# donydchen/matchnerf

Hardware: AMD Instinct MI355X
Metric: rendered rays/sec (3-view, 64 samples/ray) (higher is better)
Workload: dtype f32; 1 GPU

## Files before the change

### include/mnerf.h

```cpp
#ifndef MNERF_H_
#define MNERF_H_

#include <stdint.h>

#ifdef __cplusplus
extern "C" {
#endif

#define MNERF_ABI_VERSION 12
#define MNERF_MAX_VIEWS 16
#define MNERF_FEAT_CH 128
#define MNERF_COND_STRIDE_MAX 96
#define MNERF_COND_STRIDE_MAX_F32 64

enum {
  MNERF_OK = 0,
  MNERF_E_NULL = -1,
  MNERF_E_RANGE = -2,
  MNERF_E_UNSUPPORTED = -3,
  MNERF_E_ALIGN = -4
};

typedef struct mnerf_view {
  float extr[12];
// ... 167 lines not shown
int mnerf_window_attention_backward(const float* q, const float* k, const float* v, const float* out, const float* g_out,
                                    float* g_q, float* g_k, float* g_v, int32_t batch, int32_t h, int32_t w,
                                    int32_t num_splits, int32_t shifted, void* workspace, size_t workspace_bytes,
                                    void* stream);
int mnerf_window_attention_presplit_stats(const float* q, const float* k, const float* v, float* out, float* row_stats,
                                          int32_t batch, int32_t h, int32_t w, int32_t num_splits, int32_t shifted,
                                          void* workspace, size_t workspace_bytes, void* stream);
int mnerf_window_attention_backward_stats(const float* q, const float* k, const float* v, const float* out, const float* g_out,
                                          const float* row_stats, float* g_q, float* g_k, float* g_v, int32_t batch, int32_t h,
                                          int32_t w, int32_t num_splits, int32_t shifted, void* workspace,
                                          size_t workspace_bytes, void* stream);

int mnerf_instance_norm(const float* x, const float* residual, float* out, int64_t planes, int64_t plane_size,
                        float eps, int32_t relu_inner, int32_t relu_outer, float* out_absmax, void* stream);

int mnerf_instance_norm_backward(const float* x, const float* dy, float* dx, int64_t planes, int64_t plane_size, float eps,
                                 int32_t relu, void* stream);

int mnerf_upsample_bilinear2x(const float* in, const float* add, float* out, int64_t planes, int32_t h, int32_t w, void* stream);
int mnerf_upsample_bilinear2x_backward(const float* dout, float* din, int64_t planes, int32_t h, int32_t w, void* stream);

#define MNERF_ABSMAX_SLOTS 64
#define MNERF_ABSMAX_STRIDE 32
#define MNERF_ABSMAX_FLOATS (MNERF_ABSMAX_SLOTS * MNERF_ABSMAX_STRIDE)
typedef struct mnerf_conv {
  const float* wstream;
  int64_t wstream_floats;
  const float* bias;
  int32_t c_in, c_out, ksize, stride;
  int32_t ew;
  float leaky_slope;
} mnerf_conv;
int64_t mnerf_conv_wstream_floats(int32_t c_in, int32_t c_out, int32_t ksize);
#define MNERF_CONV_OUT_NCHW 0
#define MNERF_CONV_OUT_CHANNEL_LAST 1
#define MNERF_CONV_OUT_PAIR_MAJOR 2
int mnerf_conv2d(const mnerf_conv* cv, const float* in, int32_t in_channels_last, int32_t upsample2x,
                 const float* in_absmax, const float* add_bilinear2x, const float* add_channel_last, float* out,
                 int32_t out_layout, float* out_absmax, int32_t n_img, int32_t h_in, int32_t w_in, void* stream);
int64_t mnerf_conv_stem_wstream_floats(void);
int mnerf_conv_stem(const float* wstream, int32_t ew, const float* in, const float* in_absmax, float* out,
                    int32_t n_img, int32_t h_in, int32_t w_in, void* stream);
int mnerf_absmax(const float* x, int64_t n, float* out, void* stream);

int mnerf_conv2d_backward_data(const float* dy, const float* w_tap_major, float* dx, int32_t n_img, int32_t c_in, int32_t c_out,
                               int32_t h_in, int32_t w_in, int32_t ksize, int32_t stride, void* stream);
size_t mnerf_conv2d_backward_weight_workspace_bytes(int32_t n_img, int32_t c_in, int32_t c_out, int32_t h_in, int32_t w_in,
                                                    int32_t ksize, int32_t stride);
int mnerf_conv2d_backward_weight(const float* x, const float* dy, float* dw, void* workspace, size_t workspace_bytes, int32_t n_img,
                                 int32_t c_in, int32_t c_out, int32_t h_in, int32_t w_in, int32_t ksize, int32_t stride, void* stream);
int mnerf_conv2d_backward_weight_f16x3(const float* x, const float* dy, const float* x_absmax, const float* dy_absmax, float* dw,
                                       void* workspace, size_t workspace_bytes, int32_t n_img, int32_t c_in, int32_t c_out, int32_t h_in,
                                       int32_t w_in, int32_t ksize, int32_t stride, void* stream);
int mnerf_conv2d_forward_f32(const float* x, const float* w_tap_major, const float* bias, float* y, int32_t n_img, int32_t c_in,
                             int32_t c_out, int32_t h_in, int32_t w_in, int32_t ksize, int32_t stride, void* stream);
size_t mnerf_conv_stem_backward_weight_workspace_bytes(int32_t n_img, int32_t h_in, int32_t w_in);
int mnerf_conv_stem_backward_weight(const float* x, const float* dy, float* dw, void* workspace, size_t workspace_bytes, int32_t n_img,
// ... 89 lines not shown
```

### matchnerf_amd/csrc/conv.hip

```cpp
#include "split_f16.hpp"

#define CONV_NW 4
#define CONV_BUF_BYTES 36864u

#ifdef CONV_TIMELINE
#define CONV_TL_POINTS 6
#define CONV_TL_ITERS 64
#define CONV_TL_STAMP(k)                                                                                       \
  do {                                                                                                         \
    __builtin_amdgcn_sched_barrier(0);                                                                         \
    if (tl_out && iter < CONV_TL_ITERS) tl_out[iter * CONV_TL_POINTS + (k)] = __builtin_amdgcn_s_memtime();    \
    __builtin_amdgcn_sched_barrier(0);                                                                         \
  } while (0)
#else
#define CONV_TL_STAMP(k) do {} while (0)
#endif
struct ConvParams {
  unsigned long long* tl;
  const float* in;
  const float* wstream;
  const float* bias;
  float* out;
  const float* in_absmax;
  float* out_absmax;
// ... 320 lines not shown
  p.out_layout = out_layout;
  p.add_cl = add_channel_last;
  MNERF_REQUIRE(out_layout == MNERF_CONV_OUT_NCHW || mnerf_aligned16(out), MNERF_E_ALIGN,
                "%s: a channel-last output must be 16-byte aligned", who);
  MNERF_REQUIRE(out_layout != MNERF_CONV_OUT_PAIR_MAJOR || n_img % 2 == 0, MNERF_E_RANGE,
                "%s: pair-major output needs an even number of images, got %d", who, n_img);
  MNERF_REQUIRE(!add_channel_last || (out_layout != MNERF_CONV_OUT_NCHW && mnerf_aligned16(add_channel_last)), MNERF_E_RANGE,
                "%s: add_channel_last needs a channel-last output layout and a 16-byte aligned tile", who);
  const long long n_pix = (long long)n_img * p.h_out * p.w_out;
  const int tpw = (n_pix + 255) / 256 >= 256 ? 2 : 1;
  const long long per_wg = 32 * tpw * CONV_NW;
  const dim3 grid((unsigned)((n_pix + per_wg - 1) / per_wg));
  const size_t lds = 2 * CONV_BUF_BYTES;
  hipStream_t st = (hipStream_t)stream;
  const bool cl = in_channels_last != 0;
  MNERF_REQUIRE(!cl || nmb == 4, MNERF_E_UNSUPPORTED, "%s: channel-last input is built for c_out = 128 only", who);
#define CONV_CASE(NMB, TPW, CLV)                                                                                      \
  if (nmb == NMB && tpw == TPW && cl == CLV) {                                                                        \
    static std::atomic<unsigned long long> attr{0};                                                                   \
    if (mnerf_once_per_device(attr))                                                                                  \
      (void)hipFuncSetAttribute((const void*)conv_kernel<NMB, TPW, CLV>, hipFuncAttributeMaxDynamicSharedMemorySize,   \
                                (int)lds);                                                                            \
    hipLaunchKernelGGL((conv_kernel<NMB, TPW, CLV>), grid, dim3(CONV_NW * 64), lds, st, p);                           \
  }
  CONV_CASE(2, 2, false) CONV_CASE(2, 1, false) CONV_CASE(3, 2, false) CONV_CASE(3, 1, false)
  CONV_CASE(4, 2, false) CONV_CASE(4, 1, false) CONV_CASE(4, 2, true) CONV_CASE(4, 1, true)
#undef CONV_CASE
  return mnerf_check_launch(who);
}

#define STEM_STEPS 10
#define STEM_K 147
#define STEM_W_BYTES (STEM_STEPS * 2 * H16_UNIT_BYTES)

struct StemParams {
  const float* in;
  const float* wstream;
  float* out;
  const float* in_absmax;
  int n_img, h_in, w_in, h_out, w_out, ew;
};

__global__ __launch_bounds__(CONV_NW * 64, 2) void conv_stem_kernel(StemParams P) {
  extern __shared__ __attribute__((aligned(16))) float stem_smem[];
  const unsigned buf0 = (unsigned)(size_t)(__attribute__((address_space(3))) float*)stem_smem;
  int* tab_off = reinterpret_cast<int*>(stem_smem) + STEM_W_BYTES / 4;
  int* tab_dy = tab_off + 16 * STEM_STEPS;
  int* tab_dx = tab_dy + 16 * STEM_STEPS;
  const int tid = threadIdx.x, lane = tid & 63;
  const int wave = __builtin_amdgcn_readfirstlane(tid >> 6);
  const int n = lane & 31, hl = lane >> 5;
  {
    const float* src = P.wstream + lane * 4;
    glds_segment(src, buf0, STEM_W_BYTES / 1024, wave, CONV_NW);
  }
  const int hw_in = P.h_in * P.w_in;
  for (int k = tid; k < 16 * STEM_STEPS; k += CONV_NW * 64) {
    const int tap = k / 3, c = k - 3 * tap, dy = tap / 7 - 3, dx = tap % 7 - 3;
    const bool real = k < STEM_K;
    tab_off[k] = real ? c * hw_in + dy * P.w_in + dx : 0;
    tab_dy[k] = real ? dy : 100;
    tab_dx[k] = real ? dx : 100;
  }
  const int hw_out = P.h_out * P.w_out;
  const long long n_pix = (long long)P.n_img * hw_out;
  constexpr int TPW = 2;
  int cy[TPW], cx[TPW];
  long long ibase[TPW], obase[TPW];
  bool live[TPW];
#pragma unroll
  for (int t = 0; t < TPW; ++t) {
    const long long p = ((long long)blockIdx.x * CONV_NW + wave) * (32 * TPW) + t * 32 + n;
    live[t] = p < n_pix;
    const long long pc = live[t] ? p : n_pix - 1;
    const int img = (int)(pc / hw_out), rem = (int)(pc - (long long)img * hw_out);
    const int oy = rem / P.w_out, ox = rem - oy * P.w_out;
    cy[t] = 2 * oy;
    cx[t] = 2 * ox;
    ibase[t] = (long long)img * 3 * hw_in + (long long)cy[t] * P.w_in + cx[t];
    obase[t] = (long long)img * 64 * hw_out + rem;
  }
  const int eg = gain_exp(mnerf_absmax_read(P.in_absmax));
  const float mult = pow2i(eg);
  f32x16 acc[TPW][2];
#pragma unroll
  for (int t = 0; t < TPW; ++t) acc[t][0] = acc[t][1] = (f32x16)(0.0f);
  segment_wait();
  __syncthreads();

// ... 40 lines not shown
#pragma unroll
    for (int m = 0; m < 2; ++m) {
      const f16x8 ah = __builtin_bit_cast(f16x8, a[m * 128]), al = __builtin_bit_cast(f16x8, a[m * 128 + 64]);
#pragma unroll
      for (int t = 0; t < TPW; ++t) acc[t][m] = mfma16h(ah, b[t].lo, acc[t][m]);
#pragma unroll
      for (int t = 0; t < TPW; ++t) acc[t][m] = mfma16h(al, b[t].hi, acc[t][m]);
#pragma unroll
      for (int t = 0; t < TPW; ++t) acc[t][m] = mfma16h(ah, b[t].hi, acc[t][m]);
    }
  }
  const float cm = pow2i(-(P.ew + eg));
#pragma unroll
  for (int t = 0; t < TPW; ++t) {
    if (!live[t]) continue;
#pragma unroll
    for (int m = 0; m < 2; ++m)
#pragma unroll
      for (int r = 0; r < 16; ++r)
        P.out[obase[t] + (long long)(32 * m + 8 * (r >> 2) + 4 * hl + (r & 3)) * hw_out] = acc[t][m][r] * cm;
  }
}

extern "C" int64_t mnerf_conv_stem_wstream_floats(void) { return STEM_W_BYTES / 4; }

extern "C" int mnerf_conv_stem(const float* wstream, int32_t ew, const float* in, const float* in_absmax, float* out,
                               int32_t n_img, int32_t h_in, int32_t w_in, void* stream) {
  const char* who = "mnerf_conv_stem";
  MNERF_REQUIRE(n_img >= 0 && h_in >= 1 && w_in >= 1, MNERF_E_RANGE, "%s: n_img=%d h_in=%d w_in=%d", who, n_img, h_in, w_in);
  MNERF_REQUIRE((long long)3 * h_in * w_in <= 0x7fffffffLL, MNERF_E_RANGE, "%s: image too large", who);
  if (n_img == 0) return MNERF_OK;
  MNERF_REQUIRE(wstream && in && in_absmax && out, MNERF_E_NULL, "%s: NULL buffer", who);
  MNERF_REQUIRE(mnerf_aligned16(wstream), MNERF_E_ALIGN, "%s: wstream must be 16-byte aligned", who);
  StemParams p;
  p.in = in;
  p.wstream = wstream;
  p.out = out;
  p.in_absmax = in_absmax;
  p.n_img = n_img;
  p.h_in = h_in;
  p.w_in = w_in;
  p.h_out = (h_in + 6 - 7) / 2 + 1;
  p.w_out = (w_in + 6 - 7) / 2 + 1;
  p.ew = ew;
  const long long n_pix = (long long)n_img * p.h_out * p.w_out;
  const size_t lds = STEM_W_BYTES + 3 * 16 * STEM_STEPS * sizeof(int);
  static std::atomic<unsigned long long> attr{0};
  if (mnerf_once_per_device(attr))
    (void)hipFuncSetAttribute((const void*)conv_stem_kernel, hipFuncAttributeMaxDynamicSharedMemorySize, (int)lds);
  hipLaunchKernelGGL(conv_stem_kernel, dim3((unsigned)((n_pix + 255) / 256)), dim3(CONV_NW * 64), lds, (hipStream_t)stream, p);
  return mnerf_check_launch(who);
}
```

### matchnerf_amd/csrc/instance_norm.hip

```cpp
#include "common.hpp"

template <int THREADS>
__device__ __forceinline__ float in_block_sum(float v, float* red) {
#pragma unroll
  for (int off = 32; off > 0; off >>= 1) v += __shfl_xor(v, off, 64);
  const int wave = threadIdx.x >> 6;
  __syncthreads();
  if ((threadIdx.x & 63) == 0) red[wave] = v;
  __syncthreads();
  float t = 0.0f;
#pragma unroll
  for (int i = 0; i < THREADS / 64; ++i) t += red[i];
  return t;
}

__device__ __forceinline__ float in_finish(float x, float mean, float rstd, float res, bool has_res, int relu_inner,
                                           int relu_outer) {
  float v = (x - mean) * rstd;
  if (relu_inner) v = fmaxf(v, 0.0f);
  if (has_res) v += res;
  if (relu_outer) v = fmaxf(v, 0.0f);
  return v;
}

// ... 106 lines not shown
  const bool vec = (n & 3) == 0 && mnerf_aligned16(x) && mnerf_aligned16(out) && (!residual || mnerf_aligned16(residual));
  const dim3 grid((unsigned)planes);
#define IN_LAUNCH(T, V)                                                                                              \
  hipLaunchKernelGGL((instance_norm_cached_kernel<T, V>), grid, dim3(T), 0, st, x, residual, out, n, eps, relu_inner, \
                     relu_outer, out_absmax)
  if (vec && n <= 256 * 8 * 4) IN_LAUNCH(256, 8);
  else if (vec && n <= 256 * 20 * 4) IN_LAUNCH(256, 20);
  else if (vec && n <= 512 * 40 * 4) IN_LAUNCH(512, 40);
  else
    hipLaunchKernelGGL(instance_norm_stream_kernel, grid, dim3(256), 0, st, x, residual, out, n, eps, relu_inner, relu_outer,
                       out_absmax);
#undef IN_LAUNCH
  return mnerf_check_launch("mnerf_instance_norm");
}

__global__ __launch_bounds__(512) void instance_norm_backward_kernel(const float* __restrict__ x, const float* __restrict__ dy, float* __restrict__ dx,
                                                                     int plane_size, float eps, int relu) {
  __shared__ float red[8];
  const size_t base = (size_t)blockIdx.x * plane_size;
  const float* xs = x + base;
  const float* gs = dy + base;
  const float inv_n = 1.0f / (float)plane_size;
  float s = 0.0f;
  for (int j = threadIdx.x; j < plane_size; j += 512) s += xs[j];
  const float mean = in_block_sum<512>(s, red) * inv_n;
  float q = 0.0f;
  for (int j = threadIdx.x; j < plane_size; j += 512) {
    const float a = xs[j] - mean;
    q += a * a;
  }
// ... 178 lines not shown
```

### matchnerf_amd/gmflow.py

```python
import math
import os

import torch
import torch.nn as nn
import torch.nn.functional as F

from . import hip
from .autograd import window_attention
from .camera import pair_list


def _fused_norm(x):
    return x.is_cuda and not torch.is_grad_enabled()


def _train_hip(x):
    import os
    return (x.is_cuda and x.dtype == torch.float32 and torch.is_grad_enabled()
            and os.environ.get("MNERF_TRAIN_CNN", "hip") != "torch")


def _train_packs(owner, convs, device):
    import os
    if os.environ.get("MNERF_TRAIN_CNN", "hip") == "f32":
# ... 58 lines not shown
    return hip.conv2d(x, ws, bias, conv.in_channels, conv.out_channels, conv.kernel_size[0], conv.stride[0], ew, in_absmax, **kw)


class ResidualBlock(nn.Module):

    def __init__(self, in_planes, planes, stride=1):
        super().__init__()
        self.conv1 = nn.Conv2d(in_planes, planes, 3, stride=stride, padding=1, bias=False)
        self.conv2 = nn.Conv2d(planes, planes, 3, padding=1, bias=False)
        self.stride = stride
        if stride != 1 or in_planes != planes:
            self.downsample = nn.Sequential(nn.Conv2d(in_planes, planes, 1, stride=stride))
        else:
            self.downsample = None

    def forward_fused(self, x, x_absmax, scal):
        y = _hip_conv(self.conv1, x, x_absmax)
        hip.instance_norm(y, relu_inner=True, out=y, out_absmax=scal[0])
        y = _hip_conv(self.conv2, y, scal[0])
        if self.downsample is not None:
            x = _hip_conv(self.downsample[0], x, x_absmax)
            hip.instance_norm(x, out=x)
        hip.instance_norm(y, residual=x, relu_inner=True, relu_outer=True, out=y, out_absmax=scal[1])
        return y, scal[1]

    def forward(self, x):
        if _train_hip(x):
            from . import autograd as AG
            y = AG.instance_norm(AG.conv2d(self.conv1, x), relu=True)
            y = AG.instance_norm(AG.conv2d(self.conv2, y), relu=True)
            if self.downsample is not None:
                x = AG.instance_norm(AG.conv2d(self.downsample[0], x))
            return F.relu(x + y)
        y = F.relu(F.instance_norm(self.conv1(x)))
        y = F.relu(F.instance_norm(self.conv2(y)))
        if self.downsample is not None:
            x = F.instance_norm(self.downsample(x))
        return F.relu(x + y)


class CNNEncoder(nn.Module):

    def __init__(self, output_dim=128):
        super().__init__()
        self.conv1 = nn.Conv2d(3, 64, 7, stride=2, padding=3, bias=False)
        self.layer1 = nn.Sequential(ResidualBlock(64, 64, 1), ResidualBlock(64, 64, 1))
        self.layer2 = nn.Sequential(ResidualBlock(64, 96, 2), ResidualBlock(96, 96, 1))
        self.layer3 = nn.Sequential(ResidualBlock(96, 128, 2), ResidualBlock(128, 128, 1))
        self.conv2 = nn.Conv2d(128, output_dim, 1)
        for m in self.modules():
            if isinstance(m, nn.Conv2d):
                nn.init.kaiming_normal_(m.weight, mode="fan_out", nonlinearity="relu")

    def forward(self, x, tokens_plus=None):
        if _fused_norm(x):
            scal = hip.absmax_regions(14, x.device)
            x = x.contiguous()
            hip.absmax(x, scal[13])
            key = (int(self.conv1.weight._version), int(self.conv1.weight.data_ptr()), str(x.device))
            if getattr(self, "_stem_pack", None) is None or self._stem_pack[0] != key:
                ws, ew = pack_conv_stem(self.conv1.weight)
                self._stem_pack = (key, torch.from_numpy(ws).to(x.device), ew)
            x = hip.conv_stem(x, self._stem_pack[1], self._stem_pack[2], scal[13])
            hip.instance_norm(x, relu_inner=True, out=x, out_absmax=scal[0])
            amax, k = scal[0], 1
            for layer in (self.layer1, self.layer2, self.layer3):
                for blk in layer:
                    x, amax = blk.forward_fused(x, amax, scal[k:k + 2])
                    k += 2
            if tokens_plus is not None:
                return _hip_conv(self.conv2, x, amax, out_layout=hip.CONV_OUT_CHANNEL_LAST, add_channel_last=tokens_plus)
            return _hip_conv(self.conv2, x, amax)
        if _train_hip(x):
            from . import autograd as AG
            convs = [m for m in self.modules() if isinstance(m, nn.Conv2d)]
            _train_packs(self, convs, x.device)
            x = AG.instance_norm(AG.conv2d(self.conv1, x), relu=True)
            x = AG.conv2d(self.conv2, self.layer3(self.layer2(self.layer1(x))))
            _drop_train_packs(convs)
        else:
            x = F.relu(F.instance_norm(self.conv1(x)))
            x = self.conv2(self.layer3(self.layer2(self.layer1(x))))
        return x if tokens_plus is None else x.permute(0, 2, 3, 1) + tokens_plus.reshape(x.shape[2], x.shape[3], -1)


EB_SEG_FLOATS = 32 * 256
EB_CHUNK = 128
# ... 251 lines not shown
            else:
                right = F.interpolate(right, scale_factor=2, mode="bilinear", align_corners=False) + conv(self.conv_l2rs[i + 1], left)
        if _train_hip(x):
            _drop_train_packs(list(self.conv_ls) + list(self.conv_l2rs))
        return right


_SINE_CACHE = {}
_PAIR_INDEX_CACHE = {}


def _pair_index_tensors(v, device):
    key = (int(v), str(device))
    if key not in _PAIR_INDEX_CACHE:
        pairs = pair_list(v)
        _PAIR_INDEX_CACHE[key] = (torch.tensor([a for a, _ in pairs], device=device),
                                  torch.tensor([bb for _, bb in pairs], device=device))
    return _PAIR_INDEX_CACHE[key]


def sine_position_tokens(h, w, channels, device):
    key = (h, w, channels, str(device))
    if key not in _SINE_CACHE:
        npf = channels // 2
        y = (torch.arange(1, h + 1, dtype=torch.float32) / (h + 1e-6) * (2 * math.pi))[:, None].expand(h, w)
        x = (torch.arange(1, w + 1, dtype=torch.float32) / (w + 1e-6) * (2 * math.pi))[None, :].expand(h, w)
        i = torch.arange(npf, dtype=torch.float32)
        dim_t = 10000.0 ** (2 * torch.div(i, 2, rounding_mode="trunc") / npf)

        def emb(t):
            a = t[..., None] / dim_t
            return torch.stack([a[..., 0::2].sin(), a[..., 1::2].cos()], -1).flatten(-2)
# ... 56 lines not shown
        pe = sine_position_tokens(h // splits, w // splits, ch, x.device).repeat(splits, splits, 1).reshape(h * w, ch).contiguous()
        tok = self.backbone((x - self._mean) / self._std, tokens_plus=pe)
        if tuple(tok.shape[1:]) != (h, w, ch):
            raise ValueError(f"backbone output {tuple(tok.shape[1:])} != expected {(h, w, ch)} for a {hh}x{ww} input")
        return tok.reshape(b, n_v, h, w, ch)

    def pair_maps(self, tokens, pairs=None, attn_splits_list=None, wo_self_attn=False):
        b, v, h, w, ch = tokens.shape
        splits = self._splits(attn_splits_list)
        pairs_all = pair_list(v)
        p0, p_n = self._contiguous_range(pairs, len(pairs_all), "pair_maps pairs")
        if p_n == 0:
            up = 2 ** self.featup_net.n_blocks
            return [tokens.new_empty(b, 0, 2, h, w, ch), tokens.new_empty(b, 0, 2, up * h, up * w, ch)]
        tok = tokens.reshape(b, v, h * w, ch)
        ia, ib = _pair_index_tensors(v, tok.device)
        if p_n != len(pairs_all):
            ia, ib = ia[p0:p0 + p_n], ib[p0:p0 + p_n]
        outs0, outs1 = [], []
        for bi in range(b):
            src = torch.cat([tok[bi, ia], tok[bi, ib]], 0).contiguous()
            src = self.transformer(src, p_n, h, w, splits, wo_self_attn)
            outs0.append(torch.stack([src[:p_n], src[p_n:]], 1).reshape(p_n, 2, h, w, ch))
            if _fused_norm(src) and self.featup_net.n_blocks >= 1:
                outs1.append(self.featup_net.forward_tokens(src.reshape(2 * p_n, h, w, ch), pair_major=True))
            else:
                up = self.featup_net(src.reshape(2 * p_n, h, w, ch).permute(0, 3, 1, 2))
                up = up.permute(0, 2, 3, 1)
                outs1.append(torch.stack([up[:p_n], up[p_n:]], 1).contiguous())
        if b == 1:
            return [outs0[0].unsqueeze(0).contiguous(), outs1[0].unsqueeze(0).contiguous()]
        return [torch.stack(outs0, 0).contiguous(), torch.stack(outs1, 0).contiguous()]


def pair_major_to_view_chunks(feat_pm):
    b, p_n = feat_pm.shape[:2]
# ... 7 lines not shown
```

### matchnerf_amd/hip.py

```python
import contextlib
import ctypes as C
import os

import numpy as np

MNERF_ABI_VERSION = 12
MNERF_POSE_FLOATS = 24
MNERF_OK, MNERF_E_NULL, MNERF_E_RANGE, MNERF_E_UNSUPPORTED, MNERF_E_ALIGN = 0, -1, -2, -3, -4
MNERF_MAX_VIEWS = 16
MNERF_COND_STRIDE_MAX, MNERF_COND_STRIDE_MAX_F32 = 96, 64
SMALL_FIXED = 32

_LIB = None
_LIB_PATH = os.environ.get("MNERF_LIB") or os.path.join(os.path.dirname(os.path.abspath(__file__)), "libmnerf_hip.so")

EXPORTS = ("mnerf_abi_version", "mnerf_last_error", "mnerf_struct_size", "mnerf_ray_samples", "mnerf_composite", "mnerf_cost_volume",
           "mnerf_cost_volume_operand_bytes", "mnerf_cost_volume_operands",
           "mnerf_composite_backward", "mnerf_cost_volume_backward", "mnerf_decoder_backward", "mnerf_decoder_backward_workspace_bytes", "mnerf_debug_set_knob",
           "mnerf_decoder_wstream_floats", "mnerf_decoder_chunk", "mnerf_decoder_samples", "mnerf_render_workspace_bytes",
           "mnerf_render_chunk", "mnerf_render_chunk_fused", "mnerf_render_chunk_is_fused", "mnerf_render_takes_pose_table", "mnerf_window_attention",
           "mnerf_window_attention_presplit", "mnerf_window_attention_workspace_bytes", "mnerf_window_attention_backward", "mnerf_window_attention_backward_workspace_bytes", "mnerf_qkv_projection", "mnerf_qkv_wstream_floats", "mnerf_qkv_window_images", "mnerf_window_attention_images", "mnerf_instance_norm", "mnerf_instance_norm_backward", "mnerf_upsample_bilinear2x", "mnerf_upsample_bilinear2x_backward", "mnerf_conv2d", "mnerf_conv_wstream_floats", "mnerf_conv_stem", "mnerf_conv_stem_wstream_floats", "mnerf_absmax", "mnerf_conv2d_backward_data", "mnerf_conv2d_backward_weight", "mnerf_conv2d_backward_weight_workspace_bytes", "mnerf_conv2d_backward_weight_f16x3", "mnerf_conv2d_forward_f32", "mnerf_conv_stem_backward_weight", "mnerf_conv_stem_backward_weight_workspace_bytes", "mnerf_encoder_block", "mnerf_encoder_block_wstream_floats",
           "mnerf_encoder_layer_backward", "mnerf_encoder_layer_backward_workspace_bytes", "mnerf_qkv_backward", "mnerf_debug_gemm",
           "mnerf_window_attention_presplit_stats", "mnerf_window_attention_backward_stats", "mnerf_encoder_block_save", "mnerf_encoder_layer_backward_saved",
           "mnerf_optim_row_blocks", "mnerf_grad_sumsq", "mnerf_adamw_step", "mnerf_l2_loss",
           "mnerf_grad_bucket_floats", "mnerf_grad_pack", "mnerf_grad_unpack",
           "mnerf_image_metrics_workspace_bytes", "mnerf_image_metrics")


class MnerfError(RuntimeError):
    pass


class View(C.Structure):
    _fields_ = [("extr", C.c_float * 12), ("intr", C.c_float * 9), ("near_", C.c_float), ("far_", C.c_float)]


# ... 144 lines not shown
    lib.mnerf_window_attention_backward.argtypes = [fp, fp, fp, fp, fp, fp, fp, fp, i32, i32, i32, i32, i32, vp, C.c_size_t, vp]
    lib.mnerf_qkv_wstream_floats.restype = i64
    lib.mnerf_qkv_wstream_floats.argtypes = []
    lib.mnerf_qkv_projection.restype = C.c_int
    lib.mnerf_qkv_projection.argtypes = [fp, C.POINTER(C.c_int32), fp, fp, i32, fp, fp, fp, i32, i32, vp]
    lib.mnerf_qkv_window_images.restype = C.c_int
    lib.mnerf_qkv_window_images.argtypes = [fp, C.POINTER(C.c_int32), fp, fp, i32, fp, vp, C.c_size_t, i32, i32, i32, i32, i32, vp]
    lib.mnerf_window_attention_images.restype = C.c_int
    lib.mnerf_window_attention_images.argtypes = [fp, fp, i32, i32, i32, i32, i32, vp, C.c_size_t, vp]
    lib.mnerf_instance_norm.restype = C.c_int
    lib.mnerf_instance_norm.argtypes = [fp, fp, fp, i64, i64, C.c_float, i32, i32, fp, vp]
    lib.mnerf_upsample_bilinear2x.restype = C.c_int
    lib.mnerf_upsample_bilinear2x.argtypes = [fp, fp, fp, i64, i32, i32, vp]
    lib.mnerf_upsample_bilinear2x_backward.restype = C.c_int
    lib.mnerf_upsample_bilinear2x_backward.argtypes = [fp, fp, i64, i32, i32, vp]
    lib.mnerf_instance_norm_backward.restype = C.c_int
    lib.mnerf_instance_norm_backward.argtypes = [fp, fp, fp, i64, i64, C.c_float, i32, vp]
    lib.mnerf_conv_wstream_floats.restype = i64
    lib.mnerf_conv_wstream_floats.argtypes = [i32, i32, i32]
    lib.mnerf_conv2d.restype = C.c_int
    lib.mnerf_conv2d.argtypes = [C.POINTER(ConvLayer), fp, i32, i32, fp, fp, fp, fp, i32, fp, i32, i32, i32, vp]
    lib.mnerf_conv2d_backward_data.restype = C.c_int
    lib.mnerf_conv2d_backward_data.argtypes = [fp, fp, fp, i32, i32, i32, i32, i32, i32, i32, vp]
    lib.mnerf_conv2d_backward_weight_workspace_bytes.restype = C.c_size_t
    lib.mnerf_conv2d_backward_weight_workspace_bytes.argtypes = [i32, i32, i32, i32, i32, i32, i32]
    lib.mnerf_conv2d_backward_weight.restype = C.c_int
    lib.mnerf_conv2d_backward_weight.argtypes = [fp, fp, fp, vp, C.c_size_t, i32, i32, i32, i32, i32, i32, i32, vp]
    lib.mnerf_conv2d_backward_weight_f16x3.restype = C.c_int
    lib.mnerf_conv2d_backward_weight_f16x3.argtypes = [fp, fp, fp, fp, fp, vp, C.c_size_t, i32, i32, i32, i32, i32, i32, i32, vp]
    lib.mnerf_conv2d_forward_f32.restype = C.c_int
    lib.mnerf_conv2d_forward_f32.argtypes = [fp, fp, fp, fp, i32, i32, i32, i32, i32, i32, i32, vp]
    lib.mnerf_conv_stem_backward_weight_workspace_bytes.restype = C.c_size_t
    lib.mnerf_conv_stem_backward_weight_workspace_bytes.argtypes = [i32, i32, i32]
    lib.mnerf_conv_stem_backward_weight.restype = C.c_int
    lib.mnerf_conv_stem_backward_weight.argtypes = [fp, fp, fp, vp, C.c_size_t, i32, i32, i32, vp]
    lib.mnerf_conv_stem_wstream_floats.restype = i64
    lib.mnerf_conv_stem_wstream_floats.argtypes = []
    lib.mnerf_conv_stem.restype = C.c_int
    lib.mnerf_conv_stem.argtypes = [fp, i32, fp, fp, fp, i32, i32, i32, vp]
    lib.mnerf_absmax.restype = C.c_int
    lib.mnerf_absmax.argtypes = [fp, i64, fp, vp]
    lib.mnerf_encoder_block_wstream_floats.restype = i64
    lib.mnerf_encoder_block_wstream_floats.argtypes = [i32]
    lib.mnerf_encoder_block.restype = C.c_int
    lib.mnerf_encoder_block.argtypes = [C.POINTER(EncoderLayer), fp, fp, fp, i32, vp]
    lib.mnerf_encoder_layer_backward_workspace_bytes.restype = i64
    lib.mnerf_encoder_layer_backward_workspace_bytes.argtypes = [i32]
    lib.mnerf_encoder_layer_backward.restype = C.c_int
    lib.mnerf_encoder_layer_backward.argtypes = [C.POINTER(EncoderLayerTrain), fp, fp, fp, fp, fp, i32, vp, vp]
    lib.mnerf_qkv_backward.restype = C.c_int
    lib.mnerf_qkv_backward.argtypes = [fp] * 13 + [i32, vp]
    lib.mnerf_optim_row_blocks.restype = i64
    lib.mnerf_optim_row_blocks.argtypes = [i64]
    lib.mnerf_grad_sumsq.restype = C.c_int
# ... 609 lines not shown
    if x.dim() != 4:
        raise MnerfError(f"instance_norm: expected [N,C,H,W], got {tuple(x.shape)}")
    if residual is not None:
        _f32c(residual, "residual")
        if residual.shape != x.shape:
            raise MnerfError(f"instance_norm: residual {tuple(residual.shape)} vs x {tuple(x.shape)}")
    if out is None:
        out = torch.empty_like(x)
    n, c, h, w = x.shape
    with _on(x.device, stream) as st:
        check(lib.mnerf_instance_norm(_ptr(x), _ptr(residual), _ptr(out), n * c, h * w, float(eps), int(bool(relu_inner)),
                                      int(bool(relu_outer)), _ptr(out_absmax), st), "mnerf_instance_norm")
    return out


def absmax_regions(n, device):
    import torch
    return torch.zeros(n, ABSMAX_FLOATS, device=device, dtype=torch.float32)


def absmax_value(region):
    return region.max()


def absmax(x, out, stream=None):
    lib = load()
    _f32c(x, "x")
    with _on(x.device, stream) as st:
        check(lib.mnerf_absmax(_ptr(x), x.numel(), _ptr(out), st), "mnerf_absmax")
    return out
# ... 90 lines not shown
    nbytes = int(lib.mnerf_conv2d_backward_weight_workspace_bytes(n, c_in, c_out, h, w, int(ksize), int(stride)))
    ws = torch.empty(max(nbytes, 16), dtype=torch.uint8, device=x.device)
    if stream is not None:
        ws.record_stream(stream)
    dw = torch.empty(c_out, c_in, ksize, ksize, device=x.device, dtype=torch.float32)
    with _on(x.device, stream) as st:
        if x_absmax is not None and dy_absmax is not None:
            check(lib.mnerf_conv2d_backward_weight_f16x3(_ptr(x), _ptr(dy), _ptr(x_absmax), _ptr(dy_absmax), _ptr(dw), ws.data_ptr(), nbytes, n,
                                                         c_in, c_out, h, w, int(ksize), int(stride), st), "mnerf_conv2d_backward_weight_f16x3")
        else:
            check(lib.mnerf_conv2d_backward_weight(_ptr(x), _ptr(dy), _ptr(dw), ws.data_ptr(), nbytes, n, c_in, c_out, h, w, int(ksize),
                                                   int(stride), st), "mnerf_conv2d_backward_weight")
    return dw


def conv_stem(x, wstream, ew, in_absmax, out=None, stream=None):
    import torch
    lib = load()
    _f32c(x, "x"), _f32c(wstream, "wstream")
    if x.dim() != 4 or x.shape[1] != 3:
        raise MnerfError(f"conv_stem: expected [N,3,H,W], got {tuple(x.shape)}")
    if wstream.numel() != lib.mnerf_conv_stem_wstream_floats():
        raise MnerfError(f"conv_stem: wstream has {wstream.numel()} floats, expected {lib.mnerf_conv_stem_wstream_floats()}")
    n, _, h, w = x.shape
    if out is None:
        out = torch.empty(n, 64, (h - 1) // 2 + 1, (w - 1) // 2 + 1, device=x.device, dtype=torch.float32)
    with _on(x.device, stream) as st:
        check(lib.mnerf_conv_stem(_ptr(wstream), int(ew), _ptr(x), _ptr(in_absmax), _ptr(out), n, h, w, st), "mnerf_conv_stem")
    return out


def conv2d(x, wstream, bias, c_in, c_out, ksize, stride, ew, in_absmax, leaky=1.0, channels_last=False, upsample2x=False,
           add_bilinear2x=None, out_layout=CONV_OUT_NCHW, add_channel_last=None, out_absmax=None, out=None, stream=None):
    import torch
    lib = load()
    _f32c(x, "x"), _f32c(wstream, "wstream")
    if x.dim() != 4:
        raise MnerfError(f"conv2d: expected a 4-D tensor, got {tuple(x.shape)}")
    n, h, w = (x.shape[0], x.shape[1], x.shape[2]) if channels_last else (x.shape[0], x.shape[2], x.shape[3])
    if (x.shape[3] if channels_last else x.shape[1]) != c_in:
        raise MnerfError(f"conv2d: input {tuple(x.shape)} does not have {c_in} channels")
    up = 1 if upsample2x else 0
    pad = ksize // 2
# ... 184 lines not shown
```

Baseline: 13.14 million rays/s.

## Run CNN encoder end-to-end in channel-last layout with new instance norm

Switches the inference CNN encoder to keep activations channel-last from the stem convolution through every residual block. It adds a channel-last output path to the stem kernel, enables channel-last input convolutions for all output-channel counts, and adds a three-pass slab-parallel instance norm for NHWC tensors that uses a workspace for partial sums. The goal is to drop NCHW-strided accesses and layout mismatches between the conv and norm kernels. In exchange, each norm now takes three launches plus workspace allocations, and the conv kernel gains more template instantiations. A separate change uses index_select with a cached combined index in no-grad mode to gather pair tokens.

```diff
diff --git a/include/mnerf.h b/include/mnerf.h
--- a/include/mnerf.h
+++ b/include/mnerf.h
@@ -205,6 +205,11 @@
 int mnerf_instance_norm(const float* x, const float* residual, float* out, int64_t planes, int64_t plane_size,
                         float eps, int32_t relu_inner, int32_t relu_outer, float* out_absmax, void* stream);
 
+size_t mnerf_instance_norm_cl_workspace_bytes(int64_t n_img, int64_t plane_size, int32_t c);
+int mnerf_instance_norm_cl(const float* x, const float* residual, float* out, int64_t n_img, int64_t plane_size, int32_t c, float eps,
+                           int32_t relu_inner, int32_t relu_outer, float* out_absmax, void* workspace, size_t workspace_bytes,
+                           void* stream);
+
 int mnerf_instance_norm_backward(const float* x, const float* dy, float* dx, int64_t planes, int64_t plane_size, float eps,
                                  int32_t relu, void* stream);
 
@@ -232,6 +237,8 @@
 int64_t mnerf_conv_stem_wstream_floats(void);
 int mnerf_conv_stem(const float* wstream, int32_t ew, const float* in, const float* in_absmax, float* out,
                     int32_t n_img, int32_t h_in, int32_t w_in, void* stream);
+int mnerf_conv_stem_layout(const float* wstream, int32_t ew, const float* in, const float* in_absmax, float* out,
+                           int32_t out_layout, int32_t n_img, int32_t h_in, int32_t w_in, void* stream);
 int mnerf_absmax(const float* x, int64_t n, float* out, void* stream);
 
 int mnerf_conv2d_backward_data(const float* dy, const float* w_tap_major, float* dx, int32_t n_img, int32_t c_in, int32_t c_out,
diff --git a/matchnerf_amd/csrc/conv.hip b/matchnerf_amd/csrc/conv.hip
--- a/matchnerf_amd/csrc/conv.hip
+++ b/matchnerf_amd/csrc/conv.hip
@@ -358,7 +358,7 @@
   const size_t lds = 2 * CONV_BUF_BYTES;
   hipStream_t st = (hipStream_t)stream;
   const bool cl = in_channels_last != 0;
-  MNERF_REQUIRE(!cl || nmb == 4, MNERF_E_UNSUPPORTED, "%s: channel-last input is built for c_out = 128 only", who);
+  MNERF_REQUIRE(!cl || mnerf_aligned16(in), MNERF_E_ALIGN, "%s: a channel-last input must be 16-byte aligned", who);
 #define CONV_CASE(NMB, TPW, CLV)                                                                                      \
   if (nmb == NMB && tpw == TPW && cl == CLV) {                                                                        \
     static std::atomic<unsigned long long> attr{0};                                                                   \
@@ -368,7 +368,9 @@
     hipLaunchKernelGGL((conv_kernel<NMB, TPW, CLV>), grid, dim3(CONV_NW * 64), lds, st, p);                           \
   }
   CONV_CASE(2, 2, false) CONV_CASE(2, 1, false) CONV_CASE(3, 2, false) CONV_CASE(3, 1, false)
-  CONV_CASE(4, 2, false) CONV_CASE(4, 1, false) CONV_CASE(4, 2, true) CONV_CASE(4, 1, true)
+  CONV_CASE(4, 2, false) CONV_CASE(4, 1, false)
+  CONV_CASE(2, 2, true) CONV_CASE(2, 1, true) CONV_CASE(3, 2, true) CONV_CASE(3, 1, true)
+  CONV_CASE(4, 2, true) CONV_CASE(4, 1, true)
 #undef CONV_CASE
   return mnerf_check_launch(who);
 }
@@ -383,6 +385,7 @@
   float* out;
   const float* in_absmax;
   int n_img, h_in, w_in, h_out, w_out, ew;
+  int out_cl;
 };
 
 __global__ __launch_bounds__(CONV_NW * 64, 2) void conv_stem_kernel(StemParams P) {
@@ -410,13 +413,14 @@
   const long long n_pix = (long long)P.n_img * hw_out;
   constexpr int TPW = 2;
   int cy[TPW], cx[TPW];
-  long long ibase[TPW], obase[TPW];
+  long long ibase[TPW], obase[TPW], opix[TPW];
   bool live[TPW];
 #pragma unroll
   for (int t = 0; t < TPW; ++t) {
     const long long p = ((long long)blockIdx.x * CONV_NW + wave) * (32 * TPW) + t * 32 + n;
     live[t] = p < n_pix;
     const long long pc = live[t] ? p : n_pix - 1;
+    opix[t] = pc;
     const int img = (int)(pc / hw_out), rem = (int)(pc - (long long)img * hw_out);
     const int oy = rem / P.w_out, ox = rem - oy * P.w_out;
     cy[t] = 2 * oy;
@@ -487,6 +491,15 @@
 #pragma unroll
   for (int t = 0; t < TPW; ++t) {
     if (!live[t]) continue;
+    if (P.out_cl) {
+#pragma unroll
+      for (int m = 0; m < 2; ++m)
+#pragma unroll
+        for (int g = 0; g < 4; ++g)
+          *reinterpret_cast<float4*>(P.out + opix[t] * 64 + 32 * m + 8 * g + 4 * hl) =
+              make_float4(acc[t][m][4 * g] * cm, acc[t][m][4 * g + 1] * cm, acc[t][m][4 * g + 2] * cm, acc[t][m][4 * g + 3] * cm);
+      continue;
+    }
 #pragma unroll
     for (int m = 0; m < 2; ++m)
 #pragma unroll
@@ -499,12 +512,21 @@
 
 extern "C" int mnerf_conv_stem(const float* wstream, int32_t ew, const float* in, const float* in_absmax, float* out,
                                int32_t n_img, int32_t h_in, int32_t w_in, void* stream) {
-  const char* who = "mnerf_conv_stem";
+  return mnerf_conv_stem_layout(wstream, ew, in, in_absmax, out, MNERF_CONV_OUT_NCHW, n_img, h_in, w_in, stream);
+}
+
+extern "C" int mnerf_conv_stem_layout(const float* wstream, int32_t ew, const float* in, const float* in_absmax, float* out,
+                                      int32_t out_layout, int32_t n_img, int32_t h_in, int32_t w_in, void* stream) {
+  const char* who = "mnerf_conv_stem_layout";
+  MNERF_REQUIRE(out_layout == MNERF_CONV_OUT_NCHW || out_layout == MNERF_CONV_OUT_CHANNEL_LAST, MNERF_E_RANGE, "%s: out_layout=%d", who,
+                out_layout);
   MNERF_REQUIRE(n_img >= 0 && h_in >= 1 && w_in >= 1, MNERF_E_RANGE, "%s: n_img=%d h_in=%d w_in=%d", who, n_img, h_in, w_in);
   MNERF_REQUIRE((long long)3 * h_in * w_in <= 0x7fffffffLL, MNERF_E_RANGE, "%s: image too large", who);
   if (n_img == 0) return MNERF_OK;
   MNERF_REQUIRE(wstream && in && in_absmax && out, MNERF_E_NULL, "%s: NULL buffer", who);
   MNERF_REQUIRE(mnerf_aligned16(wstream), MNERF_E_ALIGN, "%s: wstream must be 16-byte aligned", who);
+  MNERF_REQUIRE(out_layout == MNERF_CONV_OUT_NCHW || mnerf_aligned16(out), MNERF_E_ALIGN, "%s: a channel-last output must be 16-byte aligned",
+                who);
   StemParams p;
   p.in = in;
   p.wstream = wstream;
@@ -516,6 +538,7 @@
   p.h_out = (h_in + 6 - 7) / 2 + 1;
   p.w_out = (w_in + 6 - 7) / 2 + 1;
   p.ew = ew;
+  p.out_cl = out_layout == MNERF_CONV_OUT_CHANNEL_LAST;
   const long long n_pix = (long long)n_img * p.h_out * p.w_out;
   const size_t lds = STEM_W_BYTES + 3 * 16 * STEM_STEPS * sizeof(int);
   static std::atomic<unsigned long long> attr{0};
diff --git a/matchnerf_amd/csrc/instance_norm.hip b/matchnerf_amd/csrc/instance_norm.hip
--- a/matchnerf_amd/csrc/instance_norm.hip
+++ b/matchnerf_amd/csrc/instance_norm.hip
@@ -144,6 +144,159 @@
   return mnerf_check_launch("mnerf_instance_norm");
 }
 
+#define INCL_THREADS 512
+#define INCL_MAX_SLABS 128
+
+struct InClParams {
+  const float* x;
+  const float* residual;
+  float* out;
+  float* part_sum;
+  float* part_sq;
+  float* out_absmax;
+  int hw, c, lanes, rows, rows_pow2, slab, n_slab;
+  float eps;
+  int relu_inner, relu_outer;
+};
+
+__device__ __forceinline__ float4 f4_add(float4 a, float4 b) { return make_float4(a.x + b.x, a.y + b.y, a.z + b.z, a.w + b.w); }
+
+__device__ __forceinline__ float4 incl_rows_sum(float4 v, float4* lds, bool active, int row, int cg, const InClParams& P) {
+  __syncthreads();
+  float4* mine = lds + row * P.lanes + cg;
+  if (active) *mine = v;
+  __syncthreads();
+  for (int s = P.rows_pow2 >> 1; s > 0; s >>= 1) {
+    if (active && row < s && row + s < P.rows) *mine = f4_add(*mine, mine[s * P.lanes]);
+    __syncthreads();
+  }
+  return active ? lds[cg] : make_float4(0.f, 0.f, 0.f, 0.f);
+}
+
+__device__ __forceinline__ float4 incl_image_sum(const float* part, float4* lds, bool active, int row, int cg, const InClParams& P) {
+  const float4* src = reinterpret_cast<const float4*>(part + (size_t)blockIdx.y * P.n_slab * P.c) + cg;
+  float4 s = make_float4(0.f, 0.f, 0.f, 0.f);
+  if (active)
+    for (int g = row; g < P.n_slab; g += P.rows) s = f4_add(s, src[(size_t)g * P.lanes]);
+  return incl_rows_sum(s, lds, active, row, cg, P);
+}
+
+template <int PASS>
+__global__ __launch_bounds__(INCL_THREADS) void instance_norm_cl_kernel(InClParams P) {
+  __shared__ float4 lds[INCL_THREADS];
+  __shared__ float red[INCL_THREADS / 64];
+  const int tid = threadIdx.x, row = tid / P.lanes, cg = tid - row * P.lanes;
+  const bool active = row < P.rows;
+  const size_t img_off = (size_t)blockIdx.y * P.hw * P.c;
+  const float4* src = reinterpret_cast<const float4*>(P.x + img_off) + cg;
+  const int p0 = blockIdx.x * P.slab, p1 = min(p0 + P.slab, P.hw);
+  const float inv_n = 1.0f / (float)P.hw;
+  float4 mean = make_float4(0.f, 0.f, 0.f, 0.f);
+  if (PASS >= 1) {
+    const float4 s = incl_image_sum(P.part_sum, lds, active, row, cg, P);
+    mean = make_float4(s.x * inv_n, s.y * inv_n, s.z * inv_n, s.w * inv_n);
+  }
+  if (PASS <= 1) {
+    float4 s = make_float4(0.f, 0.f, 0.f, 0.f);
+    if (active) {
+#pragma unroll 8
+      for (int p = p0 + row; p < p1; p += P.rows) {
+        const float4 v = src[(size_t)p * P.lanes];
+        if (PASS == 0) {
+          s = f4_add(s, v);
+        } else {
+          const float a = v.x - mean.x, b = v.y - mean.y, c = v.z - mean.z, d = v.w - mean.w;
+          s = f4_add(s, make_float4(a * a, b * b, c * c, d * d));
+        }
+      }
+    }
+    const float4 t = incl_rows_sum(s, lds, active, row, cg, P);
+    if (active && row == 0)
+      reinterpret_cast<float4*>((PASS == 0 ? P.part_sum : P.part_sq) + ((size_t)blockIdx.y * P.n_slab + blockIdx.x) * P.c)[cg] = t;
+  } else {
+    const float4 q = incl_image_sum(P.part_sq, lds, active, row, cg, P);
+    const float4 rstd = make_float4(1.0f / sqrtf(q.x * inv_n + P.eps), 1.0f / sqrtf(q.y * inv_n + P.eps), 1.0f / sqrtf(q.z * inv_n + P.eps),
+                                    1.0f / sqrtf(q.w * inv_n + P.eps));
+    const float4* res = P.residual ? reinterpret_cast<const float4*>(P.residual + img_off) + cg : nullptr;
+    float4* dst = reinterpret_cast<float4*>(P.out + img_off) + cg;
+    const int ri = P.relu_inner, ro = P.relu_outer;
+    float omax = 0.0f;
+    if (active) {
+#pragma unroll 4
+      for (int p = p0 + row; p < p1; p += P.rows) {
+        const size_t i = (size_t)p * P.lanes;
+        const float4 v = src[i];
+        const float4 r = res ? res[i] : make_float4(0.f, 0.f, 0.f, 0.f);
+        float4 o;
+        o.x = in_finish(v.x, mean.x, rstd.x, r.x, res != nullptr, ri, ro);
+        o.y = in_finish(v.y, mean.y, rstd.y, r.y, res != nullptr, ri, ro);
+        o.z = in_finish(v.z, mean.z, rstd.z, r.z, res != nullptr, ri, ro);
+        o.w = in_finish(v.w, mean.w, rstd.w, r.w, res != nullptr, ri, ro);
+        dst[i] = o;
+        omax = fmaxf(fmaxf(omax, fmaxf(fabsf(o.x), fabsf(o.y))), fmaxf(fabsf(o.z), fabsf(o.w)));
+      }
+    }
+    in_merge_absmax<INCL_THREADS>(omax, red, P.out_absmax);
+  }
+}
+
+static void incl_geometry(int64_t hw, int c, InClParams& p) {
+  p.lanes = c / 4;
+  p.rows = INCL_THREADS / p.lanes;
+  p.rows_pow2 = 1;
+  while (p.rows_pow2 < p.rows) p.rows_pow2 *= 2;
+  int64_t slab = (hw + INCL_MAX_SLABS - 1) / INCL_MAX_SLABS;
+  if (slab < 8 * p.rows) slab = 8 * p.rows;
+  slab = (slab + p.rows - 1) / p.rows * p.rows;
+  p.slab = (int)slab;
+  p.n_slab = (int)((hw + slab - 1) / slab);
+}
+
+static bool incl_shape_ok(int64_t n_img, int64_t hw, int c) {
+  return n_img >= 0 && n_img <= 65535 && hw >= 1 && hw <= 0x7fffffffLL / 4 && c >= 4 && c % 4 == 0 && c <= 4 * INCL_THREADS;
+}
+
+extern "C" size_t mnerf_instance_norm_cl_workspace_bytes(int64_t n_img, int64_t plane_size, int32_t c) {
+  if (!incl_shape_ok(n_img, plane_size, c)) return 0;
+  InClParams p;
+  incl_geometry(plane_size, c, p);
+  return (size_t)2 * (size_t)n_img * p.n_slab * c * sizeof(float);
+}
+
+extern "C" int mnerf_instance_norm_cl(const float* x, const float* residual, float* out, int64_t n_img, int64_t plane_size, int32_t c,
+                                      float eps, int32_t relu_inner, int32_t relu_outer, float* out_absmax, void* workspace,
+                                      size_t workspace_bytes, void* stream) {
+  const char* who = "mnerf_instance_norm_cl";
+  MNERF_REQUIRE(incl_shape_ok(n_img, plane_size, c), MNERF_E_RANGE, "%s: n_img=%lld plane_size=%lld c=%d (built: c %% 4 == 0, c <= %d)", who,
+                (long long)n_img, (long long)plane_size, c, 4 * INCL_THREADS);
+  MNERF_REQUIRE(eps >= 0.0f, MNERF_E_RANGE, "%s: eps=%g", who, (double)eps);
+  if (n_img == 0) return MNERF_OK;
+  MNERF_REQUIRE(x && out && workspace, MNERF_E_NULL, "%s: NULL buffer", who);
+  MNERF_REQUIRE(mnerf_aligned16(x) && mnerf_aligned16(out) && mnerf_aligned16(workspace) && (!residual || mnerf_aligned16(residual)),
+                MNERF_E_ALIGN, "%s: x, residual, out and workspace must be 16-byte aligned", who);
+  const size_t need = mnerf_instance_norm_cl_workspace_bytes(n_img, plane_size, c);
+  MNERF_REQUIRE(workspace_bytes >= need, MNERF_E_RANGE, "%s: workspace of %zu bytes, need %zu", who, workspace_bytes, need);
+  InClParams p;
+  p.x = x;
+  p.residual = residual;
+  p.out = out;
+  p.out_absmax = out_absmax;
+  p.hw = (int)plane_size;
+  p.c = c;
+  incl_geometry(plane_size, c, p);
+  p.part_sum = static_cast<float*>(workspace);
+  p.part_sq = p.part_sum + (size_t)n_img * p.n_slab * c;
+  p.eps = eps;
+  p.relu_inner = relu_inner;
+  p.relu_outer = relu_outer;
+  hipStream_t st = (hipStream_t)stream;
+  const dim3 grid((unsigned)p.n_slab, (unsigned)n_img);
+  hipLaunchKernelGGL(instance_norm_cl_kernel<0>, grid, dim3(INCL_THREADS), 0, st, p);
+  hipLaunchKernelGGL(instance_norm_cl_kernel<1>, grid, dim3(INCL_THREADS), 0, st, p);
+  hipLaunchKernelGGL(instance_norm_cl_kernel<2>, grid, dim3(INCL_THREADS), 0, st, p);
+  return mnerf_check_launch(who);
+}
+
 __global__ __launch_bounds__(512) void instance_norm_backward_kernel(const float* __restrict__ x, const float* __restrict__ dy, float* __restrict__ dx,
                                                                      int plane_size, float eps, int relu) {
   __shared__ float red[8];
diff --git a/matchnerf_amd/gmflow.py b/matchnerf_amd/gmflow.py
--- a/matchnerf_amd/gmflow.py
+++ b/matchnerf_amd/gmflow.py
@@ -96,14 +96,16 @@
         else:
             self.downsample = None
 
-    def forward_fused(self, x, x_absmax, scal):
-        y = _hip_conv(self.conv1, x, x_absmax)
-        hip.instance_norm(y, relu_inner=True, out=y, out_absmax=scal[0])
-        y = _hip_conv(self.conv2, y, scal[0])
+    def forward_fused(self, x, x_absmax, scal, channel_last=False):
+        kw = dict(channels_last=True, out_layout=hip.CONV_OUT_CHANNEL_LAST) if channel_last else {}
+        norm = hip.instance_norm_cl if channel_last else hip.instance_norm
+        y = _hip_conv(self.conv1, x, x_absmax, **kw)
+        norm(y, relu_inner=True, out=y, out_absmax=scal[0])
+        y = _hip_conv(self.conv2, y, scal[0], **kw)
         if self.downsample is not None:
-            x = _hip_conv(self.downsample[0], x, x_absmax)
-            hip.instance_norm(x, out=x)
-        hip.instance_norm(y, residual=x, relu_inner=True, relu_outer=True, out=y, out_absmax=scal[1])
+            x = _hip_conv(self.downsample[0], x, x_absmax, **kw)
+            norm(x, out=x)
+        norm(y, residual=x, relu_inner=True, relu_outer=True, out=y, out_absmax=scal[1])
         return y, scal[1]
 
     def forward(self, x):
@@ -123,6 +125,8 @@
 
 class CNNEncoder(nn.Module):
 
+    channel_last = True
+
     def __init__(self, output_dim=128):
         super().__init__()
         self.conv1 = nn.Conv2d(3, 64, 7, stride=2, padding=3, bias=False)
@@ -143,16 +147,18 @@
             if getattr(self, "_stem_pack", None) is None or self._stem_pack[0] != key:
                 ws, ew = pack_conv_stem(self.conv1.weight)
                 self._stem_pack = (key, torch.from_numpy(ws).to(x.device), ew)
-            x = hip.conv_stem(x, self._stem_pack[1], self._stem_pack[2], scal[13])
-            hip.instance_norm(x, relu_inner=True, out=x, out_absmax=scal[0])
+            cl = bool(self.channel_last)
+            x = hip.conv_stem(x, self._stem_pack[1], self._stem_pack[2], scal[13],
+                              out_layout=hip.CONV_OUT_CHANNEL_LAST if cl else hip.CONV_OUT_NCHW)
+            (hip.instance_norm_cl if cl else hip.instance_norm)(x, relu_inner=True, out=x, out_absmax=scal[0])
             amax, k = scal[0], 1
             for layer in (self.layer1, self.layer2, self.layer3):
                 for blk in layer:
-                    x, amax = blk.forward_fused(x, amax, scal[k:k + 2])
+                    x, amax = blk.forward_fused(x, amax, scal[k:k + 2], channel_last=cl)
                     k += 2
             if tokens_plus is not None:
-                return _hip_conv(self.conv2, x, amax, out_layout=hip.CONV_OUT_CHANNEL_LAST, add_channel_last=tokens_plus)
-            return _hip_conv(self.conv2, x, amax)
+                return _hip_conv(self.conv2, x, amax, channels_last=cl, out_layout=hip.CONV_OUT_CHANNEL_LAST, add_channel_last=tokens_plus)
+            return _hip_conv(self.conv2, x, amax, channels_last=cl)
         if _train_hip(x):
             from . import autograd as AG
             convs = [m for m in self.modules() if isinstance(m, nn.Conv2d)]
@@ -434,8 +440,8 @@
     key = (int(v), str(device))
     if key not in _PAIR_INDEX_CACHE:
         pairs = pair_list(v)
-        _PAIR_INDEX_CACHE[key] = (torch.tensor([a for a, _ in pairs], device=device),
-                                  torch.tensor([bb for _, bb in pairs], device=device))
+        ia, ib = torch.tensor([a for a, _ in pairs], device=device), torch.tensor([bb for _, bb in pairs], device=device)
+        _PAIR_INDEX_CACHE[key] = (ia, ib, torch.cat([ia, ib]))
     return _PAIR_INDEX_CACHE[key]
 
 
@@ -522,12 +528,15 @@
             up = 2 ** self.featup_net.n_blocks
             return [tokens.new_empty(b, 0, 2, h, w, ch), tokens.new_empty(b, 0, 2, up * h, up * w, ch)]
         tok = tokens.reshape(b, v, h * w, ch)
-        ia, ib = _pair_index_tensors(v, tok.device)
+        ia, ib, iab = _pair_index_tensors(v, tok.device)
         if p_n != len(pairs_all):
             ia, ib = ia[p0:p0 + p_n], ib[p0:p0 + p_n]
         outs0, outs1 = [], []
         for bi in range(b):
-            src = torch.cat([tok[bi, ia], tok[bi, ib]], 0).contiguous()
+            if torch.is_grad_enabled():
+                src = torch.cat([tok[bi, ia], tok[bi, ib]], 0).contiguous()
+            else:
+                src = tok[bi].index_select(0, iab if p_n == len(pairs_all) else torch.cat([ia, ib]))
             src = self.transformer(src, p_n, h, w, splits, wo_self_attn)
             outs0.append(torch.stack([src[:p_n], src[p_n:]], 1).reshape(p_n, 2, h, w, ch))
             if _fused_norm(src) and self.featup_net.n_blocks >= 1:
diff --git a/matchnerf_amd/hip.py b/matchnerf_amd/hip.py
--- a/matchnerf_amd/hip.py
+++ b/matchnerf_amd/hip.py
@@ -19,7 +19,7 @@
            "mnerf_composite_backward", "mnerf_cost_volume_backward", "mnerf_decoder_backward", "mnerf_decoder_backward_workspace_bytes", "mnerf_debug_set_knob",
            "mnerf_decoder_wstream_floats", "mnerf_decoder_chunk", "mnerf_decoder_samples", "mnerf_render_workspace_bytes",
            "mnerf_render_chunk", "mnerf_render_chunk_fused", "mnerf_render_chunk_is_fused", "mnerf_render_takes_pose_table", "mnerf_window_attention",
-           "mnerf_window_attention_presplit", "mnerf_window_attention_workspace_bytes", "mnerf_window_attention_backward", "mnerf_window_attention_backward_workspace_bytes", "mnerf_qkv_projection", "mnerf_qkv_wstream_floats", "mnerf_qkv_window_images", "mnerf_window_attention_images", "mnerf_instance_norm", "mnerf_instance_norm_backward", "mnerf_upsample_bilinear2x", "mnerf_upsample_bilinear2x_backward", "mnerf_conv2d", "mnerf_conv_wstream_floats", "mnerf_conv_stem", "mnerf_conv_stem_wstream_floats", "mnerf_absmax", "mnerf_conv2d_backward_data", "mnerf_conv2d_backward_weight", "mnerf_conv2d_backward_weight_workspace_bytes", "mnerf_conv2d_backward_weight_f16x3", "mnerf_conv2d_forward_f32", "mnerf_conv_stem_backward_weight", "mnerf_conv_stem_backward_weight_workspace_bytes", "mnerf_encoder_block", "mnerf_encoder_block_wstream_floats",
+           "mnerf_window_attention_presplit", "mnerf_window_attention_workspace_bytes", "mnerf_window_attention_backward", "mnerf_window_attention_backward_workspace_bytes", "mnerf_qkv_projection", "mnerf_qkv_wstream_floats", "mnerf_qkv_window_images", "mnerf_window_attention_images", "mnerf_instance_norm", "mnerf_instance_norm_cl", "mnerf_instance_norm_cl_workspace_bytes", "mnerf_instance_norm_backward", "mnerf_upsample_bilinear2x", "mnerf_upsample_bilinear2x_backward", "mnerf_conv2d", "mnerf_conv_wstream_floats", "mnerf_conv_stem", "mnerf_conv_stem_layout", "mnerf_conv_stem_wstream_floats", "mnerf_absmax", "mnerf_conv2d_backward_data", "mnerf_conv2d_backward_weight", "mnerf_conv2d_backward_weight_workspace_bytes", "mnerf_conv2d_backward_weight_f16x3", "mnerf_conv2d_forward_f32", "mnerf_conv_stem_backward_weight", "mnerf_conv_stem_backward_weight_workspace_bytes", "mnerf_encoder_block", "mnerf_encoder_block_wstream_floats",
            "mnerf_encoder_layer_backward", "mnerf_encoder_layer_backward_workspace_bytes", "mnerf_qkv_backward", "mnerf_debug_gemm",
            "mnerf_window_attention_presplit_stats", "mnerf_window_attention_backward_stats", "mnerf_encoder_block_save", "mnerf_encoder_layer_backward_saved",
            "mnerf_optim_row_blocks", "mnerf_grad_sumsq", "mnerf_adamw_step", "mnerf_l2_loss",
@@ -194,6 +194,10 @@
     lib.mnerf_upsample_bilinear2x.argtypes = [fp, fp, fp, i64, i32, i32, vp]
     lib.mnerf_upsample_bilinear2x_backward.restype = C.c_int
     lib.mnerf_upsample_bilinear2x_backward.argtypes = [fp, fp, i64, i32, i32, vp]
+    lib.mnerf_instance_norm_cl.restype = C.c_int
+    lib.mnerf_instance_norm_cl.argtypes = [fp, fp, fp, i64, i64, i32, C.c_float, i32, i32, fp, vp, C.c_size_t, vp]
+    lib.mnerf_instance_norm_cl_workspace_bytes.restype = C.c_size_t
+    lib.mnerf_instance_norm_cl_workspace_bytes.argtypes = [i64, i64, i32]
     lib.mnerf_instance_norm_backward.restype = C.c_int
     lib.mnerf_instance_norm_backward.argtypes = [fp, fp, fp, i64, i64, C.c_float, i32, vp]
     lib.mnerf_conv_wstream_floats.restype = i64
@@ -218,6 +222,8 @@
     lib.mnerf_conv_stem_wstream_floats.argtypes = []
     lib.mnerf_conv_stem.restype = C.c_int
     lib.mnerf_conv_stem.argtypes = [fp, i32, fp, fp, fp, i32, i32, i32, vp]
+    lib.mnerf_conv_stem_layout.restype = C.c_int
+    lib.mnerf_conv_stem_layout.argtypes = [fp, i32, fp, fp, fp, i32, i32, i32, i32, vp]
     lib.mnerf_absmax.restype = C.c_int
     lib.mnerf_absmax.argtypes = [fp, i64, fp, vp]
     lib.mnerf_encoder_block_wstream_floats.restype = i64
@@ -857,6 +863,31 @@
     return out
 
 
+def instance_norm_cl(x, residual=None, relu_inner=False, relu_outer=False, eps=1e-5, out=None, out_absmax=None, stream=None):
+    import torch
+    lib = load()
+    _f32c(x, "x")
+    if x.dim() != 4:
+        raise MnerfError(f"instance_norm_cl: expected [N,H,W,C], got {tuple(x.shape)}")
+    if residual is not None:
+        _f32c(residual, "residual")
+        if residual.shape != x.shape:
+            raise MnerfError(f"instance_norm_cl: residual {tuple(residual.shape)} vs x {tuple(x.shape)}")
+    if out is None:
+        out = torch.empty_like(x)
+    n, h, w, c = x.shape
+    nbytes = int(lib.mnerf_instance_norm_cl_workspace_bytes(n, h * w, c))
+    if n and not nbytes:
+        raise MnerfError(f"instance_norm_cl: unsupported shape {tuple(x.shape)}")
+    ws = torch.empty(max(nbytes, 16), dtype=torch.uint8, device=x.device)
+    if stream is not None:
+        ws.record_stream(stream)
+    with _on(x.device, stream) as st:
+        check(lib.mnerf_instance_norm_cl(_ptr(x), _ptr(residual), _ptr(out), n, h * w, c, float(eps), int(bool(relu_inner)),
+                                         int(bool(relu_outer)), _ptr(out_absmax), ws.data_ptr(), nbytes, st), "mnerf_instance_norm_cl")
+    return out
+
+
 def absmax_regions(n, device):
     import torch
     return torch.zeros(n, ABSMAX_FLOATS, device=device, dtype=torch.float32)
@@ -977,7 +1008,7 @@
     return dw
 
 
-def conv_stem(x, wstream, ew, in_absmax, out=None, stream=None):
+def conv_stem(x, wstream, ew, in_absmax, out=None, stream=None, out_layout=CONV_OUT_NCHW):
     import torch
     lib = load()
     _f32c(x, "x"), _f32c(wstream, "wstream")
@@ -986,10 +1017,14 @@
     if wstream.numel() != lib.mnerf_conv_stem_wstream_floats():
         raise MnerfError(f"conv_stem: wstream has {wstream.numel()} floats, expected {lib.mnerf_conv_stem_wstream_floats()}")
     n, _, h, w = x.shape
+    if out_layout not in (CONV_OUT_NCHW, CONV_OUT_CHANNEL_LAST):
+        raise MnerfError(f"conv_stem: out_layout={out_layout}")
     if out is None:
-        out = torch.empty(n, 64, (h - 1) // 2 + 1, (w - 1) // 2 + 1, device=x.device, dtype=torch.float32)
+        ho, wo = (h - 1) // 2 + 1, (w - 1) // 2 + 1
+        out = torch.empty((n, 64, ho, wo) if out_layout == CONV_OUT_NCHW else (n, ho, wo, 64), device=x.device, dtype=torch.float32)
     with _on(x.device, stream) as st:
-        check(lib.mnerf_conv_stem(_ptr(wstream), int(ew), _ptr(x), _ptr(in_absmax), _ptr(out), n, h, w, st), "mnerf_conv_stem")
+        check(lib.mnerf_conv_stem_layout(_ptr(wstream), int(ew), _ptr(x), _ptr(in_absmax), _ptr(out), int(out_layout), n, h, w, st),
+              "mnerf_conv_stem_layout")
     return out
 
 
```

Result: slower. 12.99 million rays/s (-1.2%).
